# nitishsaDire/objectDetection_ssd

Hardware: AMD Instinct MI355X
Metric: images/sec SSD300-VGG16 train step (higher is better)
Workload: dtype f32 (tensors, accumulators, loss, SGD; the Winograd-domain products of the layers with >= 256 reduction channels are formed from three EXACT bf16 limbs per f32 operand on the bf16 MFMA -- six limb products per f32 product, dropped terms <= 2^-26 -- measured no further from f64 than the f32 MFMA; SSD

## Files before the change

objectdetection_ssd_amd/csrc/winograd.hip:

```cpp
#include <cstdlib>
#include "internal.h"

namespace {

struct Lat { int D; int h0[4], w0[4]; };
__device__ __forceinline__ void lat_tile(const int (&first)[4], int D, int t, int& off, int& base) {
    off = 0;
#pragma unroll
    for (int a = 1; a < 4; ++a)
        if (a < D && t >= first[a]) off = a;
    base = 4 * (t - first[off]);
}

__global__ void wino_weight_kernel(const float* __restrict__ w, float* __restrict__ U, int Co, int Ci, int Nrows, int K, int mode) {
    const size_t total = (size_t)Nrows * K;
    for (size_t i = (size_t)blockIdx.x * blockDim.x + threadIdx.x; i < total; i += (size_t)gridDim.x * blockDim.x) {
        const int k = (int)(i % K), n = (int)(i / K);
        const int co = mode == 0 ? n : k, ci = mode == 0 ? k : n;
        float g[3][3];
#pragma unroll
        for (int r = 0; r < 3; ++r)
#pragma unroll
            for (int s = 0; s < 3; ++s)
                g[r][s] = (co < Co && ci < Ci) ? w[((size_t)co * Ci + ci) * 9 + (mode != 1 ? r * 3 + s : (2 - r) * 3 + (2 - s))] : 0.f;
        float t[4][3];
#pragma unroll
        for (int s = 0; s < 3; ++s) {
            t[0][s] = g[0][s];
            t[1][s] = 0.5f * (g[0][s] + g[1][s] + g[2][s]);
            t[2][s] = 0.5f * (g[0][s] - g[1][s] + g[2][s]);
            t[3][s] = g[2][s];
        }
#pragma unroll
        for (int r = 0; r < 4; ++r) {
            const float u0 = t[r][0], u1 = 0.5f * (t[r][0] + t[r][1] + t[r][2]), u2 = 0.5f * (t[r][0] - t[r][1] + t[r][2]), u3 = t[r][2];
            U[((size_t)(r * 4 + 0) * Nrows + n) * K + k] = u0;
            U[((size_t)(r * 4 + 1) * Nrows + n) * K + k] = u1;
            U[((size_t)(r * 4 + 2) * Nrows + n) * K + k] = u2;
            U[((size_t)(r * 4 + 3) * Nrows + n) * K + k] = u3;
        }
    }
}

__global__ __launch_bounds__(256) void wino_input_kernel(const float* __restrict__ x, float* __restrict__ V, int N, int H, int W, int C,
                                                         int TH, int TW) {
    const int C4 = C >> 2;
    const size_t tiles = (size_t)N * TH * TW, total = tiles * C4;
    for (size_t i = (size_t)blockIdx.x * 256 + threadIdx.x; i < total; i += (size_t)gridDim.x * 256) {
        const int c4 = (int)(i % C4);
        const size_t tile = i / C4;
        const int tw = (int)(tile % TW), th = (int)((tile / TW) % TH), n = (int)(tile / ((size_t)TW * TH));
        f32x4 d[4][4];
#pragma unroll
        for (int a = 0; a < 4; ++a) {
            const int ih = 2 * th - 1 + a;
#pragma unroll
            for (int b = 0; b < 4; ++b) {
                const int iw = 2 * tw - 1 + b;
                const bool ok = (unsigned)ih < (unsigned)H && (unsigned)iw < (unsigned)W;
                d[a][b] = ok ? *reinterpret_cast<const f32x4*>(x + (((size_t)n * H + ih) * W + iw) * C + c4 * 4) : f32x4{0.f, 0.f, 0.f, 0.f};
            }
        }
        f32x4 t[4][4];
#pragma unroll
// ... 239 lines not shown
    colsum_final4_body(part, db, nblk, C, ldp, (int)blockIdx.x);
}
struct BiasTail { const float* part; float* db; int nblk, C, ldp; };
int g_bias_tail = 1;

__device__ constexpr float W4_BT[6][6] = {{4, 0, -5, 0, 1, 0}, {0, -4, -4, 1, 1, 0}, {0, 4, -4, -1, 1, 0},
                                          {0, -2, -1, 2, 1, 0}, {0, 2, -1, -2, 1, 0}, {0, 4, 0, -5, 0, 1}};
__device__ constexpr float W4_G[6][3] = {{0.25f, 0, 0}, {-1.f / 6, -1.f / 6, -1.f / 6}, {-1.f / 6, 1.f / 6, -1.f / 6},
                                         {1.f / 24, 1.f / 12, 1.f / 6}, {1.f / 24, -1.f / 12, 1.f / 6}, {0, 0, 1}};
__device__ constexpr float W4_AT[4][6] = {{1, 1, 1, 1, 1, 0}, {0, 1, -1, 2, -2, 0}, {0, 1, 1, 4, 4, 0}, {0, 1, -1, 8, -8, 1}};
__device__ __forceinline__ float w4_g_dot(int row, float x0, float x1, float x2) {
    return __builtin_fmaf(W4_G[row][2], x2, __builtin_fmaf(W4_G[row][1], x1, W4_G[row][0] * x0));
}

__device__ __forceinline__ void store_u(float* __restrict__ U, int x3, int p, int n, int k, int Nrows, int K, float v) {
    if (!x3) {
        U[((size_t)p * Nrows + n) * K + k] = v;
        return;
    }
    const __bf16 h = (__bf16)v;
    const float r1 = v - (float)h;
    const __bf16 m = (__bf16)r1;
    const size_t limb = (size_t)((Nrows + 127) / 128 * 128) * 16;
    __bf16* d = reinterpret_cast<__bf16*>(U) + ((size_t)p * (K >> 4) + (k >> 4)) * 3 * limb + (size_t)n * 16 + (k & 15);
    d[0] = h;
    d[limb] = m;
    d[2 * limb] = (__bf16)(r1 - (float)m);
}

__global__ void wino4_weight_kernel(const float* __restrict__ w, float* __restrict__ U, int Co, int Ci, int Nrows, int K, int mode, int x3) {
    const size_t total = (size_t)Nrows * K;
    for (size_t i = (size_t)blockIdx.x * blockDim.x + threadIdx.x; i < total; i += (size_t)gridDim.x * blockDim.x) {
        const int k = (int)(i % K), n = (int)(i / K);
        const int co = mode == 0 ? n : k, ci = mode == 0 ? k : n;
        float g[3][3];
#pragma unroll
        for (int r = 0; r < 3; ++r)
#pragma unroll
            for (int s = 0; s < 3; ++s)
                g[r][s] = (co < Co && ci < Ci) ? w[((size_t)co * Ci + ci) * 9 + (mode != 1 ? r * 3 + s : (2 - r) * 3 + (2 - s))] : 0.f;
        float t[6][3];
#pragma unroll
        for (int a = 0; a < 6; ++a)
#pragma unroll
            for (int s = 0; s < 3; ++s) t[a][s] = w4_g_dot(a, g[0][s], g[1][s], g[2][s]);
#pragma unroll
        for (int a = 0; a < 6; ++a)
#pragma unroll
            for (int b = 0; b < 6; ++b)
                store_u(U, x3, a * 6 + b, n, k, Nrows, K, w4_g_dot(b, t[a][0], t[a][1], t[a][2]));
    }
}

__global__ __launch_bounds__(256) void wino4_input_kernel(const float* __restrict__ x, float* __restrict__ V, int N, int H, int W, int C,
                                                          int TH, int TW, unsigned long long* __restrict__ bits, const Lat lat) {
    const int C4 = C >> 2;
    const size_t tiles = (size_t)N * TH * TW, total = tiles * C4;
    const size_t plane = tiles * C;
    for (size_t i = (size_t)blockIdx.x * 256 + threadIdx.x; i < total; i += (size_t)gridDim.x * 256) {
        const int c4 = (int)(i % C4);
        const size_t tile = i / C4;
        const int tw = (int)(tile % TW), th = (int)((tile / TW) % TH), n = (int)(tile / ((size_t)TW * TH));
        int offh, bh, offw, bw;
        lat_tile(lat.h0, lat.D, th, offh, bh);
        lat_tile(lat.w0, lat.D, tw, offw, bw);
        f32x4 t[6][6];
        unsigned long long word = 0ull;
#pragma unroll
        for (int b = 0; b < 6; ++b) {
            f32x4 d[6];
            const int lw = bw - 1 + b, iw = lat.D * lw + offw;
#pragma unroll
            for (int a = 0; a < 6; ++a) {
                const int lh = bh - 1 + a, ih = lat.D * lh + offh;
                const bool ok = lh >= 0 && lw >= 0 && ih < H && iw < W;
                d[a] = ok ? *reinterpret_cast<const f32x4*>(x + (((size_t)n * H + ih) * W + iw) * C + c4 * 4) : f32x4{0.f, 0.f, 0.f, 0.f};
                if (a >= 1 && a <= 4 && b >= 1 && b <= 4) {
#pragma unroll
                    for (int e = 0; e < 4; ++e) word |= (unsigned long long)(d[a][e] > 0.f) << (((a - 1) * 4 + (b - 1)) * 4 + e);
                }
            }
#pragma unroll
            for (int a = 0; a < 6; ++a) {
                f32x4 acc = {0.f, 0.f, 0.f, 0.f};
#pragma unroll
                for (int k = 0; k < 6; ++k)
                    if (W4_BT[a][k] != 0.f) acc += W4_BT[a][k] * d[k];
                t[a][b] = acc;
            }
        }
        float* dst = V + tile * C + c4 * 4;
#pragma unroll
        for (int a = 0; a < 6; ++a)
#pragma unroll
            for (int b = 0; b < 6; ++b) {
                f32x4 acc = {0.f, 0.f, 0.f, 0.f};
#pragma unroll
                for (int k = 0; k < 6; ++k)
                    if (W4_BT[b][k] != 0.f) acc += W4_BT[b][k] * t[a][k];
                *reinterpret_cast<f32x4*>(dst + (size_t)(a * 6 + b) * plane) = acc;
            }
        if (bits != nullptr) bits[i] = word;
    }
}

__global__ __launch_bounds__(256) void wino4_output_kernel(const float* __restrict__ Mx, float* __restrict__ out, int N, int H, int W, int C,
                                                           int Cvalid, int ldo, int TH, int TW, const float* __restrict__ bias,
                                                           const float* __restrict__ mask, int relu, int accumulate,
                                                           const unsigned long long* __restrict__ mask_bits, const Lat lat) {
    const int C4 = C >> 2;
    const size_t tiles = (size_t)N * TH * TW, total = tiles * C4;
    const size_t plane = tiles * C;
    for (size_t i = (size_t)blockIdx.x * 256 + threadIdx.x; i < total; i += (size_t)gridDim.x * 256) {
        const int c4 = (int)(i % C4);
        const size_t tile = i / C4;
        const int tw = (int)(tile % TW), th = (int)((tile / TW) % TH), n = (int)(tile / ((size_t)TW * TH));
        int offh, bh, offw, bw;
        lat_tile(lat.h0, lat.D, th, offh, bh);
        lat_tile(lat.w0, lat.D, tw, offw, bw);
        const float* src = Mx + tile * C + c4 * 4;
        f32x4 t[4][6];
#pragma unroll
        for (int b = 0; b < 6; ++b) {
            f32x4 m[6];
#pragma unroll
            for (int a = 0; a < 6; ++a) m[a] = *reinterpret_cast<const f32x4*>(src + (size_t)(a * 6 + b) * plane);
#pragma unroll
            for (int a = 0; a < 4; ++a) {
                f32x4 acc = {0.f, 0.f, 0.f, 0.f};
#pragma unroll
                for (int k = 0; k < 6; ++k)
                    if (W4_AT[a][k] != 0.f) acc += W4_AT[a][k] * m[k];
                t[a][b] = acc;
            }
        }
        const unsigned long long word = mask_bits != nullptr ? mask_bits[i] : 0ull;
        f32x4 bv = {0.f, 0.f, 0.f, 0.f};
        if (bias != nullptr) {
#pragma unroll
            for (int e = 0; e < 4; ++e) bv[e] = c4 * 4 + e < Cvalid ? bias[c4 * 4 + e] : 0.f;
        }
#pragma unroll
        for (int a = 0; a < 4; ++a) {
            const int oh = lat.D * (bh + a) + offh;
            if (oh >= H) continue;
#pragma unroll
            for (int b = 0; b < 4; ++b) {
                const int ow = lat.D * (bw + b) + offw;
                if (ow >= W) continue;
                f32x4 v = bv;
#pragma unroll
                for (int k = 0; k < 6; ++k)
// ... 109 lines not shown
        const size_t tile0 = (size_t)(blk / cgroups) * 32, tile = tile0 + tl;
        const int c4 = cg * 8 + q;
        const bool live = tile < tiles && c4 < C4;
        const int tw = live ? (int)(tile % TW) : 0, th = live ? (int)((tile / TW) % TH) : 0, n = live ? (int)(tile / ((size_t)TW * TH)) : 0;
        f32x4 t[6][6];
        constexpr int NS = MODE == 0 ? 6 : 4;
#pragma unroll
        for (int b2 = 0; b2 < NS; ++b2) {
            f32x4 d[NS];
#pragma unroll
            for (int a = 0; a < NS; ++a) {
                const int ih = MODE == 0 ? 4 * th - 1 + a : 4 * th + a, iw = MODE == 0 ? 4 * tw - 1 + b2 : 4 * tw + b2;
                const bool ok = live && (unsigned)ih < (unsigned)H && (unsigned)iw < (unsigned)W;
                d[a] = ok ? *reinterpret_cast<const f32x4*>(src + (((size_t)n * H + ih) * W + iw) * C + c4 * 4) : f32x4{0.f, 0.f, 0.f, 0.f};
            }
#pragma unroll
            for (int a = 0; a < 6; ++a) {
                f32x4 acc = {0.f, 0.f, 0.f, 0.f};
#pragma unroll
                for (int k = 0; k < NS; ++k) {
                    const float cf = MODE == 0 ? W4_BT[a][k] : W4_AT[k][a];
                    if (cf != 0.f) acc += cf * d[k];
                }
                t[a][b2] = acc;
            }
        }
#pragma unroll
        for (int a = 0; a < 6; ++a) {
            __syncthreads();
#pragma unroll
            for (int b2 = 0; b2 < 6; ++b2) {
                f32x4 acc = {0.f, 0.f, 0.f, 0.f};
#pragma unroll
                for (int k = 0; k < NS; ++k) {
                    const float cf = MODE == 0 ? W4_BT[b2][k] : W4_AT[k][b2];
                    if (cf != 0.f) acc += cf * t[a][k];
                }
#pragma unroll
                for (int e = 0; e < 4; ++e) tr[b2][q * 4 + e][tl] = acc[e];
            }
            __syncthreads();
#pragma unroll
            for (int it = 0; it < 24; ++it) {
                const int row = it * 8 + (threadIdx.x >> 5), col = threadIdx.x & 31;
                const int b2 = row >> 5, cl = row & 31;
                const int c = cg * 32 + cl;
                if (c < C) dst[((size_t)(a * 6 + b2) * C + c) * Tpad + tile0 + col] = tr[b2][cl][col];
            }
        }
    }
}

struct PoolSrc { const uint8_t* am; const float* gate; int Hp, Wp; };
template <bool BIAS, bool POOLED = false>
__global__ __launch_bounds__(256) void wino4_dy_kernel(const float* __restrict__ dy, float* __restrict__ Y, int N, int H, int W, int C,
                                                       int TH, int TW, float* __restrict__ part, int Cvalid, float* __restrict__ Vd,
                                                       const PoolSrc ps, const Lat lat) {
    const int C4 = C >> 2;
    f32x4 bsum = {0.f, 0.f, 0.f, 0.f};
    const size_t tiles = (size_t)N * TH * TW, total = tiles * C4;
    const size_t plane = tiles * C;
    for (size_t i = (size_t)blockIdx.x * 256 + threadIdx.x; i < total; i += (size_t)gridDim.x * 256) {
        const int c4 = (int)(i % C4);
        const size_t tile = i / C4;
        const int tw = (int)(tile % TW), th = (int)((tile / TW) % TH), n = (int)(tile / ((size_t)TW * TH));
        int offh, bh, offw, bw;
        lat_tile(lat.h0, lat.D, th, offh, bh);
        lat_tile(lat.w0, lat.D, tw, offw, bw);
        f32x4 pg[4][4];
        uint32_t pc[4][4];
        if (POOLED) {
#pragma unroll
            for (int r = 0; r < 4; ++r)
#pragma unroll
                for (int q = 0; q < 4; ++q) {
                    const bool inner = (r == 1 || r == 2) && (q == 1 || q == 2);
                    const int ph = 2 * th - 1 + r, pw = 2 * tw - 1 + q;
                    const bool ok = (inner || Vd != nullptr) && (unsigned)ph < (unsigned)ps.Hp && (unsigned)pw < (unsigned)ps.Wp;
                    f32x4 d = {0.f, 0.f, 0.f, 0.f};
                    uint32_t a = 0xffffffffu;
                    if (ok) {
                        const size_t idx = (((size_t)n * ps.Hp + ph) * ps.Wp + pw) * C4 + c4;
                        d = *reinterpret_cast<const f32x4*>(dy + idx * 4);
                        const f32x4 yv = *reinterpret_cast<const f32x4*>(ps.gate + idx * 4);
                        a = *reinterpret_cast<const uint32_t*>(ps.am + idx * 4);
#pragma unroll
                        for (int e = 0; e < 4; ++e) d[e] = yv[e] > 0.f ? d[e] : 0.f;
                    }
                    pg[r][q] = d;
                    pc[r][q] = a;
                }
        }
        auto patch = [&](int a, int b) -> f32x4 {
            const int lh = bh - 1 + a, lw = bw - 1 + b;
            const int ih = lat.D * lh + offh, iw = lat.D * lw + offw;
            const bool ok = lh >= 0 && lw >= 0 && ih < H && iw < W;
            if (!POOLED)
                return ok ? *reinterpret_cast<const f32x4*>(dy + (((size_t)n * H + ih) * W + iw) * C + c4 * 4) : f32x4{0.f, 0.f, 0.f, 0.f};
            const int r = (a + 1) >> 1, q = (b + 1) >> 1;
            const uint32_t code = (uint32_t)(((a + 1) & 1) * 2 + ((b + 1) & 1));
            f32x4 g;
#pragma unroll
            for (int e = 0; e < 4; ++e) g[e] = (ok && ((pc[r][q] >> (8 * e)) & 0xffu) == code) ? pg[r][q][e] : 0.f;
            return g;
        };
        if (Vd != nullptr) {
            f32x4 u[6][6];
#pragma unroll
            for (int b = 0; b < 6; ++b) {
                f32x4 d[6];
#pragma unroll
                for (int a = 0; a < 6; ++a) d[a] = patch(a, b);
#pragma unroll
                for (int a = 0; a < 6; ++a) {
                    f32x4 acc = {0.f, 0.f, 0.f, 0.f};
#pragma unroll
                    for (int k = 0; k < 6; ++k)
                        if (W4_BT[a][k] != 0.f) acc += W4_BT[a][k] * d[k];
                    u[a][b] = acc;
                }
            }
            float* dv = Vd + tile * C + c4 * 4;
#pragma unroll
            for (int a = 0; a < 6; ++a)
#pragma unroll
                for (int b = 0; b < 6; ++b) {
                    f32x4 acc = {0.f, 0.f, 0.f, 0.f};
#pragma unroll
                    for (int k = 0; k < 6; ++k)
                        if (W4_BT[b][k] != 0.f) acc += W4_BT[b][k] * u[a][k];
                    *reinterpret_cast<f32x4*>(dv + (size_t)(a * 6 + b) * plane) = acc;
                }
        }
        f32x4 t[6][4];
#pragma unroll
        for (int b = 0; b < 4; ++b) {
            f32x4 d[4];
#pragma unroll
            for (int a = 0; a < 4; ++a) d[a] = patch(a + 1, b + 1);
            if (BIAS) bsum += (d[0] + d[1]) + (d[2] + d[3]);
#pragma unroll
            for (int a = 0; a < 6; ++a) {
                f32x4 acc = {0.f, 0.f, 0.f, 0.f};
#pragma unroll
                for (int k = 0; k < 4; ++k)
                    if (W4_AT[k][a] != 0.f) acc += W4_AT[k][a] * d[k];
                t[a][b] = acc;
            }
        }
        float* dst = Y + tile * C + c4 * 4;
#pragma unroll
        for (int a = 0; a < 6; ++a)
#pragma unroll
            for (int b = 0; b < 6; ++b) {
                f32x4 acc = {0.f, 0.f, 0.f, 0.f};
#pragma unroll
                for (int k = 0; k < 4; ++k)
                    if (W4_AT[k][b] != 0.f) acc += W4_AT[k][b] * t[a][k];
                *reinterpret_cast<f32x4*>(dst + (size_t)(a * 6 + b) * plane) = acc;
            }
    }
    if (BIAS) {
        __shared__ f32x4 red[256];
        red[threadIdx.x] = bsum;
        __syncthreads();
        if ((int)threadIdx.x < C4) {
            f32x4 t = red[threadIdx.x];
            for (int k = threadIdx.x + C4; k < 256; k += C4) t += red[k];
            const int c4 = (int)(((size_t)blockIdx.x * 256 + threadIdx.x) % C4);
#pragma unroll
            for (int e = 0; e < 4; ++e)
                if (c4 * 4 + e < Cvalid) part[(size_t)blockIdx.x * ((Cvalid + 3) / 4 * 4) + c4 * 4 + e] = t[e];
        }
    }
}

template <bool MAKE_Y, bool BIAS>
__global__ __launch_bounds__(256) void wino4_adj_out_kernel(const float* __restrict__ Md, int N, int H, int W, int C, int TH, int TW,
                                                            float* __restrict__ dx, int ldo, const float* __restrict__ mask,
                                                            const unsigned long long* __restrict__ mask_bits, int accumulate,
                                                            float* __restrict__ Y, float* __restrict__ part, int Cvalid) {
    const int C4 = C >> 2;
    f32x4 bsum = {0.f, 0.f, 0.f, 0.f};
    const size_t tiles = (size_t)N * TH * TW, total = tiles * C4;
    const size_t plane = tiles * C;
    for (size_t i = (size_t)blockIdx.x * 256 + threadIdx.x; i < total; i += (size_t)gridDim.x * 256) {
        const int c4 = (int)(i % C4);
        const size_t tile = i / C4;
        const int tw = (int)(tile % TW), th = (int)((tile / TW) % TH), n = (int)(tile / ((size_t)TW * TH));
        const float* src = Md + tile * C + c4 * 4;
        auto ld = [&](const float* base, int a, int b) -> f32x4 { return *reinterpret_cast<const f32x4*>(base + (size_t)(a * 6 + b) * plane); };
        auto rowx = [&](const f32x4 (&m)[6], f32x4 (&r)[4]) {
#pragma unroll
            for (int j = 0; j < 4; ++j) {
                f32x4 acc = {0.f, 0.f, 0.f, 0.f};
#pragma unroll
                for (int b = 0; b < 6; ++b)
                    if (W4_BT[b][j + 1] != 0.f) acc += W4_BT[b][j + 1] * m[b];
                r[j] = acc;
            }
        };
        f32x4 d[4][4];
#pragma unroll
        for (int a2 = 0; a2 < 4; ++a2)
#pragma unroll
            for (int b2 = 0; b2 < 4; ++b2) d[a2][b2] = f32x4{0.f, 0.f, 0.f, 0.f};
#pragma unroll
        for (int a = 0; a < 6; ++a) {
            f32x4 m[6], r[4];
#pragma unroll
            for (int b = 0; b < 6; ++b) m[b] = ld(src, a, b);
            rowx(m, r);
#pragma unroll
            for (int i2 = 0; i2 < 4; ++i2)
// ... 248 lines not shown
#pragma unroll
                for (int e = 0; e < 4; ++e) flat[e * 9 + r * 3 + s2] = acc[e];
            }
        f32x4* o = reinterpret_cast<f32x4*>(dw + i * 9);
#pragma unroll
        for (int j = 0; j < 9; ++j) o[j] = f32x4{flat[4 * j], flat[4 * j + 1], flat[4 * j + 2], flat[4 * j + 3]};
    }
}

int g_fused = -1;
int g_full = -1;
inline bool use_full(int mo, int K, int Nout) {
    if (mo != 4 || (K != 64 && K != 128) || g_full == 0 || g_fused == 0) return false;
    return g_full == 1;
}
int g_wino_x3 = -1;
inline bool use_x3(int mo, int K) {
    if (g_wino_x3 < 0) {
        const char* e = getenv("SSD_WINO_X3");
        g_wino_x3 = (e != nullptr && e[0] == '0') ? 0 : 1;
    }
    return g_wino_x3 == 1 && mo == 4 && K >= 256 && K % 32 == 0;
}
inline size_t align256(size_t v) { return (v + 255) & ~(size_t)255; }
inline bool use_fused(int mo, int K, int Nout) {
    if (mo != 4 || (K != 64 && K != 128 && K != 256) || g_fused == 0 || use_x3(mo, K)) return false;
    if (g_fused == 1) return true;
    return K <= 128;
}
int g_xform_cap = 8192;
inline int grid_for(size_t total) {
    const size_t b = (total + 255) / 256, cap = (size_t)g_xform_cap;
    return (int)(b > cap ? cap : (b == 0 ? 1 : b));
}

struct LatPlan { Lat lat; int TH, TW; };
LatPlan lat_plan(int H, int W, int D) {
    LatPlan p{};
    p.lat.D = D;
    int th = 0, tw = 0;
    for (int a = 0; a < 4; ++a) {
        p.lat.h0[a] = th;
        p.lat.w0[a] = tw;
        if (a < D) {
            const int sh = a < H ? (H - a + D - 1) / D : 0, sw = a < W ? (W - a + D - 1) / D : 0;
            th += (sh + 3) / 4;
            tw += (sw + 3) / 4;
        }
    }
    p.TH = th; p.TW = tw;
    return p;
}

void launch_dy_pass(const float* dy, float* Y, const ssd_conv_geom* g, int ldy, const LatPlan& lp, float* part, int bias_blocks, float* Vd,
                    const PoolSrc* ps, hipStream_t st) {
    const int TH = lp.TH, TW = lp.TW;
    const size_t tiles = (size_t)g->N * TH * TW;
    const PoolSrc none{nullptr, nullptr, 0, 0};
    if (bias_blocks > 0) {
        if (ps) hipLaunchKernelGGL((wino4_dy_kernel<true, true>), dim3(bias_blocks), dim3(256), 0, st, dy, Y, g->N, g->H, g->W, ldy, TH, TW, part, g->Co, Vd, *ps, lp.lat);
        else hipLaunchKernelGGL((wino4_dy_kernel<true, false>), dim3(bias_blocks), dim3(256), 0, st, dy, Y, g->N, g->H, g->W, ldy, TH, TW, part, g->Co, Vd, none, lp.lat);
    } else {
        const dim3 grid(grid_for(tiles * (ldy / 4)));
        if (ps) hipLaunchKernelGGL((wino4_dy_kernel<false, true>), grid, dim3(256), 0, st, dy, Y, g->N, g->H, g->W, ldy, TH, TW, static_cast<float*>(nullptr), 0, Vd, *ps, lp.lat);
        else hipLaunchKernelGGL((wino4_dy_kernel<false, false>), grid, dim3(256), 0, st, dy, Y, g->N, g->H, g->W, ldy, TH, TW, static_cast<float*>(nullptr), 0, Vd, none, lp.lat);
    }
}

int wino_conv(const WinoConv& c, const ssd_conv_geom* g, void* ws, size_t ws_bytes, hipStream_t st) {
    const int mo = c.mo, D = g->dil, N = g->N, H = g->H, W = g->W, Cin = c.K;
    const bool pooled = c.pooled.y != nullptr;
    if (D < 1 || D > 4 || (D > 1 && (mo != 4 || pooled))) return SSD_ERR_BAD_SHAPE;
    const LatPlan lp = lat_plan(H, W, D);
    const int TH = mo == 4 ? lp.TH : (H + mo - 1) / mo, TW = mo == 4 ? lp.TW : (W + mo - 1) / mo, P = (mo + 2) * (mo + 2);
    const size_t tiles = (size_t)N * TH * TW;
    const int Cvalid = c.U_rows;
    const int Cout = (Cvalid + 3) / 4 * 4;
    if (tiles >= (1ull << 31) || Cin % 32 != 0 || Cout > c.ldo || c.ldo % 4 != 0) return SSD_ERR_BAD_SHAPE;
    const size_t vb = align256((size_t)P * tiles * Cin * 4), mb = align256((size_t)P * tiles * Cout * 4);
    if (ws_bytes < vb + mb) return SSD_ERR_WORKSPACE;
    float* V = c.planes_keep != nullptr ? c.planes_keep : static_cast<float*>(ws);
    float* Mx = reinterpret_cast<float*>(static_cast<char*>(ws) + vb);
    if (D == 1 && c.planes == nullptr && use_full(mo, Cin, Cout))
        return ssd_internal_wino4_full(c, (int)tiles, H, W, TH, TW, st);
    if (c.planes != nullptr) V = const_cast<float*>(c.planes);
    else if (mo == 2) hipLaunchKernelGGL(wino_input_kernel, dim3(grid_for(tiles * (Cin / 4))), dim3(256), 0, st, c.in, V, N, H, W, Cin, TH, TW);
    else hipLaunchKernelGGL(wino4_input_kernel, dim3(grid_for(tiles * (Cin / 4))), dim3(256), 0, st, c.in, V, N, H, W, Cin, TH, TW, c.bits_out, lp.lat);
    SSD_CHECK_LAUNCH();
    if (c.mask_bits != nullptr && mo != 4) return SSD_ERR_BAD_SHAPE;
    if (D == 1 && use_fused(mo, Cin, Cout)) return ssd_internal_wino4_gemm_out(c, V, (int)tiles, H, W, TH, TW, st);
    if (use_x3(mo, Cin)) {
        if (int e = ssd_internal_gemm_batched_x3(V, c.U, Mx, (int)tiles, Cin, Cout, c.U_rows, P, tiles * Cin, st)) return e;
    } else if (int e = ssd_internal_gemm_batched(V, c.U, Mx, (int)tiles, Cin, Cout, c.U_rows, P, tiles * Cin, (size_t)c.U_rows * Cin, 1, st)) {
        return e;
    }
    if (pooled)
        hipLaunchKernelGGL(wino4_output_pool_kernel, dim3(grid_for(tiles * (Cout / 4))), dim3(256), 0, st, Mx, c.pooled.y, c.pooled.argmax, N, H, W,
                           Cout, TH, TW, c.bias, c.pooled.Ho, c.pooled.Wo);
    else if (mo == 2)
        hipLaunchKernelGGL(wino_output_kernel, dim3(grid_for(tiles * (Cout / 4))), dim3(256), 0, st, Mx, c.out, N, H, W, Cout, Cvalid, c.ldo, TH, TW,
                           c.bias, c.mask, c.relu, c.accumulate);
    else
        hipLaunchKernelGGL(wino4_output_kernel, dim3(grid_for(tiles * (Cout / 4))), dim3(256), 0, st, Mx, c.out, N, H, W, Cout, Cvalid, c.ldo, TH,
                           TW, c.bias, c.mask, c.relu, c.accumulate, c.mask_bits, lp.lat);
    SSD_CHECK_LAUNCH();
    return SSD_OK;
}

bool wino_geom_ok(const ssd_conv_geom* g) {
    return g && g->R == 3 && g->S == 3 && g->stride == 1 && g->dil >= 1 && g->dil <= 4 && g->pad == g->dil && g->Ho == g->H && g->Wo == g->W && g->N > 0 &&
           g->H > 0 && g->W > 0 && g->Ci > 0 && g->Co > 0;
}

}

extern "C" int ssd_wino_weights(const float* w_oihw, float* U_fwd, float* U_bwd, int Co, int Ci, int Co_pad, int mo, void* stream) {
    if (!w_oihw || (!U_fwd && !U_bwd)) return SSD_ERR_NULL;
    if (Co <= 0 || Ci <= 0 || Co_pad < Co || (mo != 2 && mo != 4)) return SSD_ERR_BAD_SHAPE;
    hipStream_t st = (hipStream_t)stream;
    if (U_fwd) {
        if (mo == 2) hipLaunchKernelGGL(wino_weight_kernel, dim3(grid_for((size_t)Co * Ci)), dim3(256), 0, st, w_oihw, U_fwd, Co, Ci, Co, Ci, 0);
        else hipLaunchKernelGGL(wino4_weight_kernel, dim3(grid_for((size_t)Co * Ci)), dim3(256), 0, st, w_oihw, U_fwd, Co, Ci, Co, Ci, 0, (int)use_x3(4, Ci));
        SSD_CHECK_LAUNCH();
    }
    if (U_bwd) {
        if (mo == 2) hipLaunchKernelGGL(wino_weight_kernel, dim3(grid_for((size_t)Ci * Co_pad)), dim3(256), 0, st, w_oihw, U_bwd, Co, Ci, Ci, Co_pad, 1);
        else hipLaunchKernelGGL(wino4_weight_kernel, dim3(grid_for((size_t)Ci * Co_pad)), dim3(256), 0, st, w_oihw, U_bwd, Co, Ci, Ci, Co_pad, 1, (int)use_x3(4, Co_pad));
        SSD_CHECK_LAUNCH();
    }
    return SSD_OK;
}

extern "C" size_t ssd_conv3x3_wino_workspace(const ssd_conv_geom* g, int direction, int mo) {
    if (!wino_geom_ok(g) || (mo != 2 && mo != 4)) return 0;
    if (mo == 2 && g->dil != 1) return 0;
    const LatPlan lp = lat_plan(g->H, g->W, g->dil);
    const size_t tiles = mo == 4 ? (size_t)g->N * lp.TH * lp.TW : (size_t)g->N * ((g->H + 1) / 2) * ((g->W + 1) / 2), P = (size_t)(mo + 2) * (mo + 2);
    const int co_pad = (g->Co + 31) / 32 * 32;
    const size_t cin = direction == 0 ? g->Ci : co_pad, cout = direction == 0 ? (size_t)(g->Co + 3) / 4 * 4 : (size_t)(g->Ci + 3) / 4 * 4;
    return align256(P * tiles * cin * 4) + align256(P * tiles * cout * 4);
// ... 237 lines not shown
    const int unit = c4 / gcd;
    int blocks = grid_for(tiles * c4);
    if (blocks > DY_BIAS_BLOCKS) blocks = DY_BIAS_BLOCKS;
    blocks = (blocks + unit - 1) / unit * unit;
    if (blocks > DY_BIAS_BLOCKS) blocks -= unit;
    return blocks;
}

int wgrad4_tail(const float* Y, const float* V, float* Zs, const float* part, int bias_blocks, float* dw, float* dbias, const ssd_conv_geom* g,
                int ldy, const WinoWgradPlan& w, bool one_call, hipStream_t st) {
    if (Y != nullptr)
        if (int e = launch_wgrad_tn(Y, V, Zs, g, ldy, w, st)) return e;
    const size_t total = (size_t)g->Co * g->Ci;
    int ks_left = w.ks;
    if (w.ks > 1 && total / 4 < 65536) {
        hipLaunchKernelGGL(wino_splitk_sum_kernel, dim3(grid_for(total / 4 * w.P)), dim3(256), 0, st, Zs, total, w.P, w.ks);
        SSD_CHECK_LAUNCH();
        ks_left = 1;
    }
    if (dbias && bias_blocks == 0 && !one_call) return SSD_ERR_BAD_SHAPE;
    const int nfin = grid_for(total / 4), ldp = (g->Co + 3) / 4 * 4;
    const bool tail = dbias && bias_blocks > 0 && (g_bias_tail || !one_call);
    const BiasTail bt{tail ? part : nullptr, dbias, bias_blocks, g->Co, ldp};
    hipLaunchKernelGGL(wino4_wgrad_finish_kernel, dim3(nfin + (tail ? (ldp + 15) / 16 : 0)), dim3(256), 0, st, Zs, dw, g->Co, g->Ci, ks_left,
                       (size_t)w.ks * total, nfin, bt);
    SSD_CHECK_LAUNCH();
    if (dbias && bias_blocks > 0 && !tail) {
        hipLaunchKernelGGL(colsum_final4_kernel, dim3((ldp + 15) / 16), dim3(256), 0, st, part, dbias, bias_blocks, g->Co, ldp);
        SSD_CHECK_LAUNCH();
    }
    return SSD_OK;
}

int wino_wgrad(const float* x, const float* planes, const float* dy, int ldy, float* dw_oihw, float* dbias, const ssd_conv_geom* g, int mo,
               float* dgrad_planes, void* workspace, size_t workspace_bytes, void* stream, const PoolSrc* pool = nullptr) {
    if (!dy || !dw_oihw || !workspace) return SSD_ERR_NULL;
    if (!wino_geom_ok(g) || g->Ci % 4 != 0 || ldy % 4 != 0 || ldy < g->Co || (mo != 2 && mo != 4)) return SSD_ERR_BAD_SHAPE;
    if (!ssd_aligned16(dy) || !ssd_aligned16(workspace) || !ssd_aligned16(dw_oihw)) return SSD_ERR_ALIGN;
    const WinoWgradPlan w = wino_wgrad_plan(g, ldy, mo);
    if (w.tiles >= (1ull << 31)) return SSD_ERR_BAD_SHAPE;
    if (workspace_bytes < w.yb + w.vb + w.zb + w.pb) return SSD_ERR_WORKSPACE;
    hipStream_t st = (hipStream_t)stream;
    char* base = static_cast<char*>(workspace);
    float* Yt = reinterpret_cast<float*>(base);
    float* Vt = reinterpret_cast<float*>(base + w.yb);
    float* Zs = reinterpret_cast<float*>(base + w.yb + w.vb);
    float* part = reinterpret_cast<float*>(base + w.yb + w.vb + w.zb);
    const bool tn = mo == 4 && (g_wgrad_tn || planes != nullptr);
    if (dgrad_planes != nullptr && !tn) return SSD_ERR_BAD_SHAPE;
    if (g->dil != 1 && (pool != nullptr || !tn)) return SSD_ERR_BAD_SHAPE;
    const int dy_bias_blocks = tn && dbias ? dy_bias_blocks_for(ldy, w.tiles) : 0;
    if (tn) {
        launch_dy_pass(dy, Yt, g, ldy, w.lp, part, dy_bias_blocks, dgrad_planes, pool, st);
        if (planes == nullptr)
            hipLaunchKernelGGL(wino4_input_kernel, dim3(grid_for(w.tiles * (g->Ci / 4))), dim3(256), 0, st, x, Vt, g->N, g->H, g->W, g->Ci, w.TH,
                               w.TW, static_cast<unsigned long long*>(nullptr), w.lp.lat);
        SSD_CHECK_LAUNCH();
        if (int e = wgrad4_tail(Yt, planes != nullptr ? planes : Vt, Zs, part, dy_bias_blocks, dw_oihw, dbias, g, ldy, w, true, st)) return e;
    } else {
        const int gy = (w.Tpad / 32) * ((ldy / 4 + 7) / 8), gx = (w.Tpad / 32) * ((g->Ci / 4 + 7) / 8);
        const dim3 gyd(gy > 16384 ? 16384 : gy), gxd(gx > 16384 ? 16384 : gx);
        if (mo == 2) {
            hipLaunchKernelGGL(wino_xform_t_kernel<1>, gyd, dim3(256), 0, st, dy, Yt, g->N, g->H, g->W, ldy, w.TH, w.TW, w.Tpad);
            hipLaunchKernelGGL(wino_xform_t_kernel<0>, gxd, dim3(256), 0, st, x, Vt, g->N, g->H, g->W, g->Ci, w.TH, w.TW, w.Tpad);
        } else {
            hipLaunchKernelGGL(wino4_xform_t_kernel<1>, gyd, dim3(256), 0, st, dy, Yt, g->N, g->H, g->W, ldy, w.TH, w.TW, w.Tpad);
            hipLaunchKernelGGL(wino4_xform_t_kernel<0>, gxd, dim3(256), 0, st, x, Vt, g->N, g->H, g->W, g->Ci, w.TH, w.TW, w.Tpad);
        }
        SSD_CHECK_LAUNCH();
        if (int e = ssd_internal_gemm_batched(Yt, Vt, Zs, g->Co, w.Tpad, g->Ci, g->Ci, w.P, (size_t)ldy * w.Tpad, (size_t)g->Ci * w.Tpad, w.ks, st))
            return e;
        if (mo == 2) {
            hipLaunchKernelGGL(wino_wgrad_finish_kernel, dim3(grid_for((size_t)g->Co * g->Ci)), dim3(256), 0, st, Zs, dw_oihw, g->Co, g->Ci, w.ks);
            SSD_CHECK_LAUNCH();
        } else if (int e = wgrad4_tail(nullptr, nullptr, Zs, part, 0, dw_oihw, dbias, g, ldy, w, true, st)) {
            return e;
        }
    }
    if (dbias && dy_bias_blocks == 0) {
        const size_t M = (size_t)g->N * g->H * g->W;
        int cq = 1;
        while (cq < (g->Co + 3) / 4 && cq < 256) cq <<= 1;
        hipLaunchKernelGGL(colsum_partial_kernel, dim3(COLSUM_BLOCKS), dim3(256), 0, st, dy, part, M, ldy, g->Co, cq);
        SSD_CHECK_LAUNCH();
        hipLaunchKernelGGL(colsum_final_kernel, dim3((g->Co + 15) / 16), dim3(256), 0, st, part, dbias, COLSUM_BLOCKS, g->Co);
        SSD_CHECK_LAUNCH();
    }
    return SSD_OK;
}
}

extern "C" int ssd_conv3x3_wino_wgrad(const float* x, const float* dy, int ldy, float* dw_oihw, float* dbias, const ssd_conv_geom* g,
                                      int mo, void* workspace, size_t workspace_bytes, void* stream) {
    if (!x) return SSD_ERR_NULL;
    if (!ssd_aligned16(x)) return SSD_ERR_ALIGN;
    return wino_wgrad(x, nullptr, dy, ldy, dw_oihw, dbias, g, mo, nullptr, workspace, workspace_bytes, stream);
}
extern "C" int ssd_conv3x3_wino_wgrad_planes(const float* planes, const float* dy, int ldy, float* dw_oihw, float* dbias,
                                             const ssd_conv_geom* g, float* dgrad_planes_out, void* workspace, size_t workspace_bytes,
                                             void* stream) {
    if (!planes) return SSD_ERR_NULL;
    if (!ssd_aligned16(planes) || (dgrad_planes_out && !ssd_aligned16(dgrad_planes_out))) return SSD_ERR_ALIGN;
    return wino_wgrad(nullptr, planes, dy, ldy, dw_oihw, dbias, g, 4, dgrad_planes_out, workspace, workspace_bytes, stream);
}

extern "C" size_t ssd_wino4_bias_partial_floats(const ssd_conv_geom* g, int ldy) {
    if (!wino_geom_ok(g) || ldy < g->Co || ldy % 4 != 0) return 0;
    return (size_t)DY_BIAS_BLOCKS * ldy;
}
// ... 323 lines not shown
```

Measured before the change: 1605.

## Use buffer-resource loads and hoisted patch loads in Winograd F4 input/dy transforms

The Winograd F(4,3) input and dy transform kernels now issue all 36 patch loads up front, followed by a scheduling barrier. When the tensor fits in 32-bit offsets, they use raw buffer loads with 32-bit offsets and hardware out-of-bounds zeroing, and launch with a two-waves-per-SIMD occupancy hint. The dy kernel also splits the Vd and non-Vd paths at compile time, so the non-Vd path loads only the inner 4x4 patch, and pooled gate/argmax loads are batched. The aim is more memory-level parallelism and cheaper address and bounds arithmetic, at the cost of higher register pressure and more template instantiations.

```diff
diff --git a/objectdetection_ssd_amd/csrc/winograd.hip b/objectdetection_ssd_amd/csrc/winograd.hip
--- a/objectdetection_ssd_amd/csrc/winograd.hip
+++ b/objectdetection_ssd_amd/csrc/winograd.hip
@@ -1,4 +1,5 @@
 #include <cstdlib>
+#include <type_traits>
 #include "internal.h"
 
 namespace {
@@ -6,10 +7,11 @@
 struct Lat { int D; int h0[4], w0[4]; };
 __device__ __forceinline__ void lat_tile(const int (&first)[4], int D, int t, int& off, int& base) {
     off = 0;
+    int f = first[0];
 #pragma unroll
     for (int a = 1; a < 4; ++a)
-        if (a < D && t >= first[a]) off = a;
-    base = 4 * (t - first[off]);
+        if (a < D && t >= first[a]) { off = a; f = first[a]; }
+    base = 4 * (t - f);
 }
 
 __global__ void wino_weight_kernel(const float* __restrict__ w, float* __restrict__ U, int Co, int Ci, int Nrows, int K, int mode) {
@@ -355,11 +357,32 @@
     }
 }
 
-__global__ __launch_bounds__(256) void wino4_input_kernel(const float* __restrict__ x, float* __restrict__ V, int N, int H, int W, int C,
-                                                          int TH, int TW, unsigned long long* __restrict__ bits, const Lat lat) {
+constexpr unsigned XF_OOB = 0xFFFFFFF0u;
+constexpr size_t XF_SRD_MAX = 0xFFFFFF00u;
+template <bool SRD> using xf_off_t = std::conditional_t<SRD, unsigned, size_t>;
+__device__ __forceinline__ __amdgpu_buffer_rsrc_t xf_srd(const void* base, size_t bytes) {
+    return __builtin_amdgcn_make_buffer_rsrc(const_cast<void*>(base), 0, (int)bytes, 0x00020000);
+}
+template <bool SRD>
+__device__ __forceinline__ f32x4 xf_load16(const void* base, __amdgpu_buffer_rsrc_t srd, xf_off_t<SRD> off, bool ok) {
+    if constexpr (SRD) return __builtin_bit_cast(f32x4, __builtin_amdgcn_raw_buffer_load_b128(srd, (int)(ok ? off : XF_OOB), 0, 0));
+    else return ok ? *reinterpret_cast<const f32x4*>(static_cast<const char*>(base) + off) : f32x4{0.f, 0.f, 0.f, 0.f};
+}
+template <bool SRD>
+__device__ __forceinline__ uint32_t xf_load4(const void* base, __amdgpu_buffer_rsrc_t srd, xf_off_t<SRD> off, bool ok) {
+    if constexpr (SRD) return (uint32_t)__builtin_amdgcn_raw_buffer_load_b32(srd, (int)(ok ? off : XF_OOB), 0, 0);
+    else return ok ? *reinterpret_cast<const uint32_t*>(static_cast<const char*>(base) + off) : 0u;
+}
+
+template <bool SRD>
+__global__ __launch_bounds__(256, SRD ? 2 : 1) void wino4_input_kernel(const float* __restrict__ x, float* __restrict__ V, int N, int H, int W, int C,
+                                                             int TH, int TW, unsigned long long* __restrict__ bits, const Lat lat) {
+    using off_t = xf_off_t<SRD>;
     const int C4 = C >> 2;
     const size_t tiles = (size_t)N * TH * TW, total = tiles * C4;
     const size_t plane = tiles * C;
+    const __amdgpu_buffer_rsrc_t srd = xf_srd(x, (size_t)N * H * W * C * 4);
+    const off_t rs = (off_t)lat.D * (off_t)W * (off_t)C * 4u, cs = (off_t)lat.D * (off_t)C * 4u;
     for (size_t i = (size_t)blockIdx.x * 256 + threadIdx.x; i < total; i += (size_t)gridDim.x * 256) {
         const int c4 = (int)(i % C4);
         const size_t tile = i / C4;
@@ -367,29 +390,40 @@
         int offh, bh, offw, bw;
         lat_tile(lat.h0, lat.D, th, offh, bh);
         lat_tile(lat.w0, lat.D, tw, offw, bw);
-        f32x4 t[6][6];
+        const off_t o00 = ((((off_t)n * (off_t)H + (off_t)(lat.D * (bh - 1) + offh)) * (off_t)W + (off_t)(lat.D * (bw - 1) + offw)) * (off_t)C +
+                           (off_t)(c4 * 4)) * 4u;
+        bool okh[6], okw[6];
+#pragma unroll
+        for (int a = 0; a < 6; ++a) {
+            const int lh = bh - 1 + a, lw = bw - 1 + a;
+            okh[a] = (lh >= 0) & (lat.D * lh + offh < H);
+            okw[a] = (lw >= 0) & (lat.D * lw + offw < W);
+        }
+        f32x4 d[6][6];
+#pragma unroll
+        for (int b = 0; b < 6; ++b)
+#pragma unroll
+            for (int a = 0; a < 6; ++a) d[a][b] = xf_load16<SRD>(x, srd, o00 + (off_t)a * rs + (off_t)b * cs, okh[a] & okw[b]);
+        __builtin_amdgcn_sched_barrier(0);
         unsigned long long word = 0ull;
 #pragma unroll
+        for (int b = 1; b <= 4; ++b)
+#pragma unroll
+            for (int a = 1; a <= 4; ++a)
+#pragma unroll
+                for (int e = 0; e < 4; ++e) word |= (unsigned long long)(d[a][b][e] > 0.f) << (((a - 1) * 4 + (b - 1)) * 4 + e);
+#pragma unroll
         for (int b = 0; b < 6; ++b) {
-            f32x4 d[6];
-            const int lw = bw - 1 + b, iw = lat.D * lw + offw;
-#pragma unroll
-            for (int a = 0; a < 6; ++a) {
-                const int lh = bh - 1 + a, ih = lat.D * lh + offh;
-                const bool ok = lh >= 0 && lw >= 0 && ih < H && iw < W;
-                d[a] = ok ? *reinterpret_cast<const f32x4*>(x + (((size_t)n * H + ih) * W + iw) * C + c4 * 4) : f32x4{0.f, 0.f, 0.f, 0.f};
-                if (a >= 1 && a <= 4 && b >= 1 && b <= 4) {
-#pragma unroll
-                    for (int e = 0; e < 4; ++e) word |= (unsigned long long)(d[a][e] > 0.f) << (((a - 1) * 4 + (b - 1)) * 4 + e);
-                }
-            }
+            f32x4 col[6];
+#pragma unroll
+            for (int a = 0; a < 6; ++a) col[a] = d[a][b];
 #pragma unroll
             for (int a = 0; a < 6; ++a) {
                 f32x4 acc = {0.f, 0.f, 0.f, 0.f};
 #pragma unroll
                 for (int k = 0; k < 6; ++k)
-                    if (W4_BT[a][k] != 0.f) acc += W4_BT[a][k] * d[k];
-                t[a][b] = acc;
+                    if (W4_BT[a][k] != 0.f) acc += W4_BT[a][k] * col[k];
+                d[a][b] = acc;
             }
         }
         float* dst = V + tile * C + c4 * 4;
@@ -400,7 +434,7 @@
                 f32x4 acc = {0.f, 0.f, 0.f, 0.f};
 #pragma unroll
                 for (int k = 0; k < 6; ++k)
-                    if (W4_BT[b][k] != 0.f) acc += W4_BT[b][k] * t[a][k];
+                    if (W4_BT[b][k] != 0.f) acc += W4_BT[b][k] * d[a][k];
                 *reinterpret_cast<f32x4*>(dst + (size_t)(a * 6 + b) * plane) = acc;
             }
         if (bits != nullptr) bits[i] = word;
@@ -616,71 +650,88 @@
 }
 
 struct PoolSrc { const uint8_t* am; const float* gate; int Hp, Wp; };
-template <bool BIAS, bool POOLED = false>
-__global__ __launch_bounds__(256) void wino4_dy_kernel(const float* __restrict__ dy, float* __restrict__ Y, int N, int H, int W, int C,
-                                                       int TH, int TW, float* __restrict__ part, int Cvalid, float* __restrict__ Vd,
-                                                       const PoolSrc ps, const Lat lat) {
+template <bool BIAS, bool POOLED, bool SRD>
+__global__ __launch_bounds__(256, SRD ? 2 : 1) void wino4_dy_kernel(const float* __restrict__ dy, float* __restrict__ Y, int N, int H, int W, int C,
+                                                          int TH, int TW, float* __restrict__ part, int Cvalid, float* __restrict__ Vd,
+                                                          const PoolSrc ps, const Lat lat) {
+    using off_t = xf_off_t<SRD>;
     const int C4 = C >> 2;
     f32x4 bsum = {0.f, 0.f, 0.f, 0.f};
     const size_t tiles = (size_t)N * TH * TW, total = tiles * C4;
     const size_t plane = tiles * C;
-    for (size_t i = (size_t)blockIdx.x * 256 + threadIdx.x; i < total; i += (size_t)gridDim.x * 256) {
+    const size_t src_bytes = POOLED ? (size_t)N * ps.Hp * ps.Wp * C * 4 : (size_t)N * H * W * C * 4;
+    const __amdgpu_buffer_rsrc_t srd_dy = xf_srd(dy, src_bytes), srd_gate = xf_srd(ps.gate, src_bytes), srd_am = xf_srd(ps.am, src_bytes / 4);
+    const off_t rs = (off_t)lat.D * (off_t)W * (off_t)C * 4u, cs = (off_t)lat.D * (off_t)C * 4u;
+    auto one = [&](auto with_vd, size_t i) {
+        constexpr bool VD = decltype(with_vd)::value;
+        constexpr int P0 = VD ? 0 : 1, P1 = VD ? 6 : 5;
         const int c4 = (int)(i % C4);
         const size_t tile = i / C4;
         const int tw = (int)(tile % TW), th = (int)((tile / TW) % TH), n = (int)(tile / ((size_t)TW * TH));
         int offh, bh, offw, bw;
         lat_tile(lat.h0, lat.D, th, offh, bh);
         lat_tile(lat.w0, lat.D, tw, offw, bw);
-        f32x4 pg[4][4];
-        uint32_t pc[4][4];
-        if (POOLED) {
-#pragma unroll
-            for (int r = 0; r < 4; ++r)
-#pragma unroll
-                for (int q = 0; q < 4; ++q) {
-                    const bool inner = (r == 1 || r == 2) && (q == 1 || q == 2);
+        bool okh[6], okw[6];
+#pragma unroll
+        for (int a = 0; a < 6; ++a) {
+            const int lh = bh - 1 + a, lw = bw - 1 + a;
+            okh[a] = (lh >= 0) & (lat.D * lh + offh < H);
+            okw[a] = (lw >= 0) & (lat.D * lw + offw < W);
+        }
+        f32x4 d[6][6];
+        if constexpr (POOLED) {
+            constexpr int Q0 = VD ? 0 : 1, Q1 = VD ? 4 : 3;
+            f32x4 pg[4][4], gt[4][4];
+            uint32_t pc[4][4];
+            const off_t i00 = (((off_t)n * (off_t)ps.Hp + (off_t)(2 * th - 1)) * (off_t)ps.Wp + (off_t)(2 * tw - 1)) * (off_t)C4 + (off_t)c4;
+            const off_t prs = (off_t)ps.Wp * (off_t)C4;
+#pragma unroll
+            for (int r = Q0; r < Q1; ++r)
+#pragma unroll
+                for (int q = Q0; q < Q1; ++q) {
                     const int ph = 2 * th - 1 + r, pw = 2 * tw - 1 + q;
-                    const bool ok = (inner || Vd != nullptr) && (unsigned)ph < (unsigned)ps.Hp && (unsigned)pw < (unsigned)ps.Wp;
-                    f32x4 d = {0.f, 0.f, 0.f, 0.f};
-                    uint32_t a = 0xffffffffu;
-                    if (ok) {
-                        const size_t idx = (((size_t)n * ps.Hp + ph) * ps.Wp + pw) * C4 + c4;
-                        d = *reinterpret_cast<const f32x4*>(dy + idx * 4);
-                        const f32x4 yv = *reinterpret_cast<const f32x4*>(ps.gate + idx * 4);
-                        a = *reinterpret_cast<const uint32_t*>(ps.am + idx * 4);
-#pragma unroll
-                        for (int e = 0; e < 4; ++e) d[e] = yv[e] > 0.f ? d[e] : 0.f;
-                    }
-                    pg[r][q] = d;
-                    pc[r][q] = a;
-                }
-        }
-        auto patch = [&](int a, int b) -> f32x4 {
-            const int lh = bh - 1 + a, lw = bw - 1 + b;
-            const int ih = lat.D * lh + offh, iw = lat.D * lw + offw;
-            const bool ok = lh >= 0 && lw >= 0 && ih < H && iw < W;
-            if (!POOLED)
-                return ok ? *reinterpret_cast<const f32x4*>(dy + (((size_t)n * H + ih) * W + iw) * C + c4 * 4) : f32x4{0.f, 0.f, 0.f, 0.f};
-            const int r = (a + 1) >> 1, q = (b + 1) >> 1;
-            const uint32_t code = (uint32_t)(((a + 1) & 1) * 2 + ((b + 1) & 1));
-            f32x4 g;
-#pragma unroll
-            for (int e = 0; e < 4; ++e) g[e] = (ok && ((pc[r][q] >> (8 * e)) & 0xffu) == code) ? pg[r][q][e] : 0.f;
-            return g;
-        };
-        if (Vd != nullptr) {
+                    const bool ok = ((unsigned)ph < (unsigned)ps.Hp) & ((unsigned)pw < (unsigned)ps.Wp);
+                    const off_t idx = i00 + (off_t)r * prs + (off_t)q * (off_t)C4;
+                    pg[r][q] = xf_load16<SRD>(dy, srd_dy, idx * 16u, ok);
+                    gt[r][q] = xf_load16<SRD>(ps.gate, srd_gate, idx * 16u, ok);
+                    pc[r][q] = xf_load4<SRD>(ps.am, srd_am, idx * 4u, ok);
+                }
+            __builtin_amdgcn_sched_barrier(0);
+#pragma unroll
+            for (int r = Q0; r < Q1; ++r)
+#pragma unroll
+                for (int q = Q0; q < Q1; ++q)
+#pragma unroll
+                    for (int e = 0; e < 4; ++e) pg[r][q][e] = gt[r][q][e] > 0.f ? pg[r][q][e] : 0.f;
+#pragma unroll
+            for (int b = P0; b < P1; ++b)
+#pragma unroll
+                for (int a = P0; a < P1; ++a) {
+                    const int r = (a + 1) >> 1, q = (b + 1) >> 1;
+                    const uint32_t code = (uint32_t)(((a + 1) & 1) * 2 + ((b + 1) & 1));
+#pragma unroll
+                    for (int e = 0; e < 4; ++e)
+                        d[a][b][e] = ((okh[a] & okw[b]) & (((pc[r][q] >> (8 * e)) & 0xffu) == code)) ? pg[r][q][e] : 0.f;
+                }
+        } else {
+            const off_t o00 = ((((off_t)n * (off_t)H + (off_t)(lat.D * (bh - 1) + offh)) * (off_t)W + (off_t)(lat.D * (bw - 1) + offw)) * (off_t)C +
+                               (off_t)(c4 * 4)) * 4u;
+#pragma unroll
+            for (int b = P0; b < P1; ++b)
+#pragma unroll
+                for (int a = P0; a < P1; ++a) d[a][b] = xf_load16<SRD>(dy, srd_dy, o00 + (off_t)a * rs + (off_t)b * cs, okh[a] & okw[b]);
+            __builtin_amdgcn_sched_barrier(0);
+        }
+        if constexpr (VD) {
             f32x4 u[6][6];
 #pragma unroll
             for (int b = 0; b < 6; ++b) {
-                f32x4 d[6];
-#pragma unroll
-                for (int a = 0; a < 6; ++a) d[a] = patch(a, b);
 #pragma unroll
                 for (int a = 0; a < 6; ++a) {
                     f32x4 acc = {0.f, 0.f, 0.f, 0.f};
 #pragma unroll
                     for (int k = 0; k < 6; ++k)
-                        if (W4_BT[a][k] != 0.f) acc += W4_BT[a][k] * d[k];
+                        if (W4_BT[a][k] != 0.f) acc += W4_BT[a][k] * d[k][b];
                     u[a][b] = acc;
                 }
             }
@@ -699,16 +750,16 @@
         f32x4 t[6][4];
 #pragma unroll
         for (int b = 0; b < 4; ++b) {
-            f32x4 d[4];
-#pragma unroll
-            for (int a = 0; a < 4; ++a) d[a] = patch(a + 1, b + 1);
-            if (BIAS) bsum += (d[0] + d[1]) + (d[2] + d[3]);
+            f32x4 blk[4];
+#pragma unroll
+            for (int a = 0; a < 4; ++a) blk[a] = d[a + 1][b + 1];
+            if (BIAS) bsum += (blk[0] + blk[1]) + (blk[2] + blk[3]);
 #pragma unroll
             for (int a = 0; a < 6; ++a) {
                 f32x4 acc = {0.f, 0.f, 0.f, 0.f};
 #pragma unroll
                 for (int k = 0; k < 4; ++k)
-                    if (W4_AT[k][a] != 0.f) acc += W4_AT[k][a] * d[k];
+                    if (W4_AT[k][a] != 0.f) acc += W4_AT[k][a] * blk[k];
                 t[a][b] = acc;
             }
         }
@@ -723,7 +774,11 @@
                     if (W4_AT[k][b] != 0.f) acc += W4_AT[k][b] * t[a][k];
                 *reinterpret_cast<f32x4*>(dst + (size_t)(a * 6 + b) * plane) = acc;
             }
-    }
+    };
+    if (Vd != nullptr)
+        for (size_t i = (size_t)blockIdx.x * 256 + threadIdx.x; i < total; i += (size_t)gridDim.x * 256) one(std::true_type{}, i);
+    else
+        for (size_t i = (size_t)blockIdx.x * 256 + threadIdx.x; i < total; i += (size_t)gridDim.x * 256) one(std::false_type{}, i);
     if (BIAS) {
         __shared__ f32x4 red[256];
         red[threadIdx.x] = bsum;
@@ -1078,18 +1133,29 @@
     return p;
 }
 
+void launch_input4(const float* x, float* V, int N, int H, int W, int C, const LatPlan& lp, unsigned long long* bits, hipStream_t st) {
+    const dim3 grid(grid_for((size_t)N * lp.TH * lp.TW * (C / 4)));
+    if ((size_t)N * H * W * C * 4 <= XF_SRD_MAX) hipLaunchKernelGGL(wino4_input_kernel<true>, grid, dim3(256), 0, st, x, V, N, H, W, C, lp.TH, lp.TW, bits, lp.lat);
+    else hipLaunchKernelGGL(wino4_input_kernel<false>, grid, dim3(256), 0, st, x, V, N, H, W, C, lp.TH, lp.TW, bits, lp.lat);
+}
+
 void launch_dy_pass(const float* dy, float* Y, const ssd_conv_geom* g, int ldy, const LatPlan& lp, float* part, int bias_blocks, float* Vd,
                     const PoolSrc* ps, hipStream_t st) {
     const int TH = lp.TH, TW = lp.TW;
     const size_t tiles = (size_t)g->N * TH * TW;
-    const PoolSrc none{nullptr, nullptr, 0, 0};
-    if (bias_blocks > 0) {
-        if (ps) hipLaunchKernelGGL((wino4_dy_kernel<true, true>), dim3(bias_blocks), dim3(256), 0, st, dy, Y, g->N, g->H, g->W, ldy, TH, TW, part, g->Co, Vd, *ps, lp.lat);
-        else hipLaunchKernelGGL((wino4_dy_kernel<true, false>), dim3(bias_blocks), dim3(256), 0, st, dy, Y, g->N, g->H, g->W, ldy, TH, TW, part, g->Co, Vd, none, lp.lat);
+    const PoolSrc src = ps ? *ps : PoolSrc{nullptr, nullptr, 0, 0};
+    const bool bias = bias_blocks > 0;
+    const dim3 grid(bias ? bias_blocks : grid_for(tiles * (ldy / 4)));
+    const int cvalid = bias ? g->Co : 0;
+    if (!bias) part = nullptr;
+    const bool srd = (ps ? (size_t)g->N * ps->Hp * ps->Wp : (size_t)g->N * g->H * g->W) * ldy * 4 <= XF_SRD_MAX;
+    auto go = [&](auto kernel) { hipLaunchKernelGGL(kernel, grid, dim3(256), 0, st, dy, Y, g->N, g->H, g->W, ldy, TH, TW, part, cvalid, Vd, src, lp.lat); };
+    if (srd) {
+        if (bias) ps ? go(wino4_dy_kernel<true, true, true>) : go(wino4_dy_kernel<true, false, true>);
+        else ps ? go(wino4_dy_kernel<false, true, true>) : go(wino4_dy_kernel<false, false, true>);
     } else {
-        const dim3 grid(grid_for(tiles * (ldy / 4)));
-        if (ps) hipLaunchKernelGGL((wino4_dy_kernel<false, true>), grid, dim3(256), 0, st, dy, Y, g->N, g->H, g->W, ldy, TH, TW, static_cast<float*>(nullptr), 0, Vd, *ps, lp.lat);
-        else hipLaunchKernelGGL((wino4_dy_kernel<false, false>), grid, dim3(256), 0, st, dy, Y, g->N, g->H, g->W, ldy, TH, TW, static_cast<float*>(nullptr), 0, Vd, none, lp.lat);
+        if (bias) ps ? go(wino4_dy_kernel<true, true, false>) : go(wino4_dy_kernel<true, false, false>);
+        else ps ? go(wino4_dy_kernel<false, true, false>) : go(wino4_dy_kernel<false, false, false>);
     }
 }
 
@@ -1111,7 +1177,7 @@
         return ssd_internal_wino4_full(c, (int)tiles, H, W, TH, TW, st);
     if (c.planes != nullptr) V = const_cast<float*>(c.planes);
     else if (mo == 2) hipLaunchKernelGGL(wino_input_kernel, dim3(grid_for(tiles * (Cin / 4))), dim3(256), 0, st, c.in, V, N, H, W, Cin, TH, TW);
-    else hipLaunchKernelGGL(wino4_input_kernel, dim3(grid_for(tiles * (Cin / 4))), dim3(256), 0, st, c.in, V, N, H, W, Cin, TH, TW, c.bits_out, lp.lat);
+    else launch_input4(c.in, V, N, H, W, Cin, lp, c.bits_out, st);
     SSD_CHECK_LAUNCH();
     if (c.mask_bits != nullptr && mo != 4) return SSD_ERR_BAD_SHAPE;
     if (D == 1 && use_fused(mo, Cin, Cout)) return ssd_internal_wino4_gemm_out(c, V, (int)tiles, H, W, TH, TW, st);
@@ -1455,9 +1521,7 @@
     const int dy_bias_blocks = tn && dbias ? dy_bias_blocks_for(ldy, w.tiles) : 0;
     if (tn) {
         launch_dy_pass(dy, Yt, g, ldy, w.lp, part, dy_bias_blocks, dgrad_planes, pool, st);
-        if (planes == nullptr)
-            hipLaunchKernelGGL(wino4_input_kernel, dim3(grid_for(w.tiles * (g->Ci / 4))), dim3(256), 0, st, x, Vt, g->N, g->H, g->W, g->Ci, w.TH,
-                               w.TW, static_cast<unsigned long long*>(nullptr), w.lp.lat);
+        if (planes == nullptr) launch_input4(x, Vt, g->N, g->H, g->W, g->Ci, w.lp, nullptr, st);
         SSD_CHECK_LAUNCH();
         if (int e = wgrad4_tail(Yt, planes != nullptr ? planes : Vt, Zs, part, dy_bias_blocks, dw_oihw, dbias, g, ldy, w, true, st)) return e;
     } else {
```

Result: faster. 1626, median of 6 (+1.3%).
